# magenta/mt3

Hardware: NVIDIA B200
Metric: audio_seconds_per_second (higher is better)
Workload: dtype f32

## Files before the change

### mt3_b200/csrc/decode.cuh

```cuda
#pragma once

#include <cuda_fp16.h>

#include "common.cuh"
#include "gemm_simt.cuh"
#include "tc.cuh"

namespace mt3 {

__device__ __forceinline__ void l2_prefetch_bulk(const void* gsrc, uint32_t bytes) {
  asm volatile("cp.async.bulk.prefetch.L2.global [%0], %1;" ::"l"(reinterpret_cast<uint64_t>(gsrc)), "r"(bytes) : "memory");
}

struct DecGemmArgs {
  const float* A; int lda;
  const float* W; int ldw;
  int M, N, K;
  int norm;
  float eps;
  int epi;
  const float* R; int ldr;
  float* C; int ldc;
  int n_split; void* C1; int kv_fmt; int hm_rows_per_b; int hm_cap; int hm_H; const int* hm_pos;
  float* partial;
// ... 101 lines not shown
      *reinterpret_cast<float4*>(mine + (ty * 4 + i) * BN + tx * 4) = make_float4(acc[i][0], acc[i][1], acc[i][2], acc[i][3]);
    if ((tid & 15) == 0) {
#pragma unroll
      for (int i = 0; i < 8; ++i) mine[BM * BN + (tid >> 4) + 8 * i] = ss[i];
    }
    __threadfence();
    __syncthreads();
    if (tid == 0) {
      const int ticket = atomicAdd(&p.counters[blockIdx.x], 1);
      s_last = (ticket == splits - 1);
      if (s_last) p.counters[blockIdx.x] = 0;
    }
    __syncthreads();
    if (!s_last) return;
    __threadfence();
#pragma unroll
    for (int i = 0; i < 4; ++i)
#pragma unroll
      for (int j = 0; j < 4; ++j) acc[i][j] = 0.f;
    float sst = 0.f;
    for (int s0 = 0; s0 < splits; s0 += 4) {
      float4 v[4][4];
      float sv[4];
#pragma unroll
      for (int u = 0; u < 4; ++u) {
        const int s = s0 + u;
        const float* src = p.partial + ((long long)min(s, splits - 1) * n_tiles + blockIdx.x) * kDecTileFloats;
#pragma unroll
        for (int i = 0; i < 4; ++i) v[u][i] = __ldcg(reinterpret_cast<const float4*>(src + (ty * 4 + i) * BN + tx * 4));
        sv[u] = (tid < BM) ? __ldcg(src + BM * BN + tid) : 0.f;
      }
#pragma unroll
      for (int u = 0; u < 4; ++u) {
        if (s0 + u < splits) {
#pragma unroll
          for (int i = 0; i < 4; ++i) {
            acc[i][0] += v[u][i].x; acc[i][1] += v[u][i].y; acc[i][2] += v[u][i].z; acc[i][3] += v[u][i].w;
          }
          sst += sv[u];
        }
      }
    }
    if (tid < BM) s_ss[tid] = sst;
  } else {
    if ((tid & 15) == 0) {
#pragma unroll
      for (int i = 0; i < 8; ++i) s_ss[(tid >> 4) + 8 * i] = ss[i];
    }
  }
  __syncthreads();

#pragma unroll
  for (int i = 0; i < 4; ++i) {
    const int m = ty * 4 + i;
    if (m >= p.M) continue;
    const int n = n0 + tx * 4;
    if (n >= p.N) continue;
    const float rs = p.norm ? 1.0f / sqrtf(s_ss[m] / (float)p.K + p.eps) : 1.f;
    float4 v = make_float4(acc[i][0] * rs, acc[i][1] * rs, acc[i][2] * rs, acc[i][3] * rs);
    if (p.epi == EPI_GATED_GELU) {
      *reinterpret_cast<float2*>(p.C + (long long)m * p.ldc + (n >> 1)) = make_float2(gelu_tanh(v.x) * v.y, gelu_tanh(v.z) * v.w);
      continue;
    }
    if (p.epi == EPI_RESIDUAL) {
      const float4 q = *reinterpret_cast<const float4*>(p.R + (long long)m * p.ldr + n);
      v.x += q.x; v.y += q.y; v.z += q.z; v.w += q.w;
    }
    dec_store4(p, m, n, v);
  }
}

__device__ __forceinline__ uint32_t cluster_map(uint32_t smem_addr, unsigned rank) {
  uint32_t r;
  asm volatile("mapa.shared::cluster.u32 %0, %1, %2;" : "=r"(r) : "r"(smem_addr), "r"(rank));
  return r;
}
__device__ __forceinline__ void st_cluster_f4(uint32_t addr, float4 v) {
  asm volatile("st.shared::cluster.v4.f32 [%0], {%1, %2, %3, %4};" ::"r"(addr), "f"(v.x), "f"(v.y), "f"(v.z), "f"(v.w) : "memory");
}
__device__ __forceinline__ void st_cluster_f1(uint32_t addr, float x) {
  asm volatile("st.shared::cluster.f32 [%0], %1;" ::"r"(addr), "f"(x) : "memory");
}

constexpr int kDecLDB = kDecBN + 8;
constexpr int kDecRedFloats = 8 * 8 * kDecBN;
template <int KC, int G>
constexpr size_t dec_cluster_smem() {
  return (size_t)(kDecBM * (KC + 4) + KC * kDecLDB + kDecRedFloats + 64 + (G > 1 ? kDecBM * kDecBN : 0)) * sizeof(float);
}

template <int S>
__device__ __forceinline__ void dec_reduce_epilogue(const DecGemmArgs& p, const float* Red, const float* Rss, unsigned rank, int n0) {
  constexpr int BN = kDecBN, R = kDecBM / S, CPT = (R * BN) / 128, LPR = BN / CPT;
  static_assert(CPT == 1 || CPT == 2, "cluster size must be 8 or 16");
  const int tid = threadIdx.x;
  const int rl = tid / LPR, c0 = (tid % LPR) * CPT;
  const int m = (int)rank * R + rl, n = n0 + c0;
  float v[2] = {0.f, 0.f};
  float sst = 0.f;
#pragma unroll
  for (int s = 0; s < S; ++s) {
    if (CPT == 2) {
      const float2 q = *reinterpret_cast<const float2*>(&Red[(s * R + rl) * BN + c0]);
      v[0] += q.x; v[1] += q.y;
    } else {
      v[0] += Red[(s * R + rl) * BN + c0];
    }
    if (p.norm) sst += Rss[s * R + rl];
  }
  const bool valid = m < p.M && n < p.N;
  if (valid) {
    const float rs = p.norm ? 1.0f / sqrtf(sst / (float)p.K + p.eps) : 1.f;
    v[0] *= rs; v[1] *= rs;
    if (CPT == 2 && p.epi == EPI_GATED_GELU) {
      p.C[(long long)m * p.ldc + (n >> 1)] = gelu_tanh(v[0]) * v[1];
    } else {
      if (p.epi == EPI_RESIDUAL) {
        const float* r = p.R + (long long)m * p.ldr + n;
        v[0] += r[0];
        if (CPT == 2) v[1] += r[1];
      }
      if (n < p.n_split) {
        float* dst = p.C + (long long)m * p.ldc + n;
        if (CPT == 2) *reinterpret_cast<float2*>(dst) = make_float2(v[0], v[1]);
        else dst[0] = v[0];
      } else {
        int d;
        char* row = reinterpret_cast<char*>(p.C1) + kv_dest(m, n - p.n_split, p.hm_rows_per_b, p.hm_cap, p.hm_H, p.hm_pos ? *p.hm_pos : 0, p.kv_fmt, d);
        kv_store<CPT>(row, p.kv_fmt, d, v);
      }
    }
  }
  if (p.ssq_out) {
    float sq = valid ? fmaf(v[0], v[0], CPT == 2 ? v[1] * v[1] : 0.f) : 0.f;
#pragma unroll
    for (int o = LPR / 2; o >= 1; o >>= 1) sq += __shfl_xor_sync(0xffffffffu, sq, o);
    if ((tid % LPR) == 0 && m < p.M) p.ssq_out[(long long)m * p.ssq_ld + n0 / BN] = sq;
  }
}

template <int KC, bool TRACE, int S, int G>
__device__ __forceinline__ void dec_cluster_body(const DecGemmArgs& p, const int tile_x) {
  constexpr int BM = kDecBM, BN = kDecBN, NT = 128 * G, LDA = KC + 4, LDB = kDecLDB;
  constexpr int R = BM / S;
  constexpr int KG = KC / G;
  static_assert(KG % 4 == 0 && (KC / (2 * G)) % 4 == 0, "K chunk must split into float4 pieces per group / per ssq thread");
  extern __shared__ __align__(16) float dsm[];
  float* As = dsm;
  float* Bs = As + BM * LDA;
  float* Red = Bs + KC * LDB;
  float* Rss = Red + kDecRedFloats;
  float* Part = Rss + 64;

  unsigned rank;
  asm volatile("mov.u32 %0, %%cluster_ctarank;" : "=r"(rank));
  const int tid = threadIdx.x;
  const int grp = tid >> 7, t128 = tid & 127;
  const int n0 = tile_x * BN;
  const int kbeg = blockIdx.y * KC;
  const bool tr = TRACE && p.trace != nullptr && tid == 0;
  const bool tr0 = tr && tile_x == 0 && blockIdx.y == 0;
  long long c0 = 0;
  if (tr) {
    atomicMin(p.trace, gtime_ns());
    c0 = clock64();
    if (tile_x == 0) {
      unsigned smid;
      asm volatile("mov.u32 %0, %%smid;" : "=r"(smid));
      if (blockIdx.y < 8) p.trace[8 + blockIdx.y] = smid;
    }
  }
  asm volatile("barrier.cluster.arrive.relaxed.aligned;" ::: "memory");

  for (int idx = tid; idx < KC * 8; idx += NT) {
    const int kr = idx >> 3, nq = idx & 7;
    const bool ok = n0 + nq * 4 < p.N;
    const float* src = p.W + (long long)(kbeg + kr) * p.ldw + (ok ? n0 + nq * 4 : 0);
    asm volatile("cp.async.cg.shared.global [%0], [%1], 16, %2;" ::"r"(tc::smem_u32(&Bs[kr * LDB + nq * 4])), "l"(src),
                 "r"(ok ? 16 : 0) : "memory");
  }
  pdl_wait();
  pdl_trigger();
  for (int idx = tid; idx < KC * 16; idx += NT) {
    const int row = idx / (KC / 4), kq = idx % (KC / 4);
    const bool ok = row < p.M;
    const int col = kbeg + kq * 4;
    const float* src = (p.A2 != nullptr && col >= p.K0) ? p.A2 + (long long)(ok ? row : 0) * p.lda2 + (col - p.K0)
                                                         : p.A + (long long)(ok ? row : 0) * p.lda + col;
    asm volatile("cp.async.cg.shared.global [%0], [%1], 16, %2;" ::"r"(tc::smem_u32(&As[row * LDA + kq * 4])), "l"(src),
                 "r"(ok ? 16 : 0) : "memory");
  }
  asm volatile("cp.async.commit_group;\n\tcp.async.wait_group 0;" ::: "memory");
  __syncthreads();
  if (tr0) p.trace[2] = (unsigned long long)(clock64() - c0);

  float ss = 0.f;
  if (p.norm) {
    constexpr int PIECE = KC / (2 * G);
    const float* ar = As + (tid / (2 * G)) * LDA + (tid % (2 * G)) * PIECE;
#pragma unroll
    for (int k = 0; k < PIECE; k += 4) {
      const float4 v = *reinterpret_cast<const float4*>(ar + k);
      ss = fmaf(v.x, v.x, ss); ss = fmaf(v.y, v.y, ss); ss = fmaf(v.z, v.z, ss); ss = fmaf(v.w, v.w, ss);
    }
    ss += __shfl_xor_sync(0xffffffffu, ss, 1);
    if (G == 2) ss += __shfl_xor_sync(0xffffffffu, ss, 2);
  }

  const int tx = t128 % 8, ty = t128 / 8;
  float2 acc[4][2];
#pragma unroll
  for (int i = 0; i < 4; ++i) acc[i][0] = acc[i][1] = make_float2(0.f, 0.f);
  {
    const float* Ag = As + grp * KG;
    const float* Bg = Bs + grp * KG * LDB;
#pragma unroll 4
    for (int k = 0; k < KG; k += 4) {
      float4 a[4], b[4];
#pragma unroll
      for (int i = 0; i < 4; ++i) a[i] = *reinterpret_cast<const float4*>(&Ag[(ty + 16 * i) * LDA + k]);
#pragma unroll
      for (int kk = 0; kk < 4; ++kk) b[kk] = *reinterpret_cast<const float4*>(&Bg[(k + kk) * LDB + tx * 4]);
#pragma unroll
      for (int i = 0; i < 4; ++i) {
        const float av[4] = {a[i].x, a[i].y, a[i].z, a[i].w};
#pragma unroll
        for (int kk = 0; kk < 4; ++kk) {
          ffma2(acc[i][0], av[kk], make_float2(b[kk].x, b[kk].y));
          ffma2(acc[i][1], av[kk], make_float2(b[kk].z, b[kk].w));
        }
      }
    }
  }
  if (G == 2) {
    if (grp == 1) {
#pragma unroll
      for (int i = 0; i < 4; ++i)
        *reinterpret_cast<float4*>(&Part[(ty + 16 * i) * BN + tx * 4]) = make_float4(acc[i][0].x, acc[i][0].y, acc[i][1].x, acc[i][1].y);
    }
    __syncthreads();
    if (grp == 0) {
#pragma unroll
      for (int i = 0; i < 4; ++i) {
        const float4 q = *reinterpret_cast<const float4*>(&Part[(ty + 16 * i) * BN + tx * 4]);
        acc[i][0].x += q.x; acc[i][0].y += q.y; acc[i][1].x += q.z; acc[i][1].y += q.w;
      }
    }
  }
  if (tr0) p.trace[3] = (unsigned long long)(clock64() - c0);
  asm volatile("barrier.cluster.wait.aligned;" ::: "memory");

  const uint32_t red_base = tc::smem_u32(Red) + rank * (R * BN * 4);
  const uint32_t rss_base = tc::smem_u32(Rss) + rank * (R * 4);
  if (grp == 0) {
#pragma unroll
    for (int i = 0; i < 4; ++i) {
      const int row = ty + 16 * i;
      st_cluster_f4(cluster_map(red_base + (uint32_t)(((row % R) * BN + tx * 4) * 4), (unsigned)(row / R)),
                    make_float4(acc[i][0].x, acc[i][0].y, acc[i][1].x, acc[i][1].y));
    }
  }
  if (p.norm && (tid % (2 * G)) == 0) {
    const int row = tid / (2 * G);
    st_cluster_f1(cluster_map(rss_base + (uint32_t)((row % R) * 4), (unsigned)(row / R)), ss);
  }
  asm volatile("barrier.cluster.arrive.release.aligned;\n\tbarrier.cluster.wait.acquire.aligned;" ::: "memory");
  if (tr0) p.trace[4] = (unsigned long long)(clock64() - c0);

  if (grp == 0) dec_reduce_epilogue<S>(p, Red, Rss, rank, n0);
  if (tr) {
    if (tr0) p.trace[5] = (unsigned long long)(clock64() - c0);
    atomicMax(p.trace + 1, gtime_ns());
  }
}

template <int KC, bool TRACE, int S, int G>
__global__ void __launch_bounds__(128 * G)
sgemm_dec_cluster_kernel(const DecGemmArgs p) {
  dec_cluster_body<KC, TRACE, S, G>(p, (int)blockIdx.x);
}

template <int KC0, int KC1, bool TRACE, int G>
__global__ void __launch_bounds__(128 * G)
sgemm_dec_cluster2_kernel(const DecGemmArgs p0, const DecGemmArgs p1, const int tiles0) {
  if ((int)blockIdx.x < tiles0) dec_cluster_body<KC0, TRACE, 8, G>(p0, (int)blockIdx.x);
  else dec_cluster_body<KC1, TRACE, 8, G>(p1, (int)blockIdx.x - tiles0);
}

constexpr int kDecGroups = 1;

template <int KC0, int KC1, int G>
inline int launch_dec_gemm_cluster2_g(const DecGemmArgs& a0, const DecGemmArgs& a1, cudaStream_t s, bool pdl) {
  constexpr size_t smem = dec_cluster_smem<(KC0 > KC1 ? KC0 : KC1), G>();
  static bool attr_done = false;
  if (!attr_done) {
    MT3_CUDA_CHECK(cudaFuncSetAttribute(sgemm_dec_cluster2_kernel<KC0, KC1, false, G>, cudaFuncAttributeMaxDynamicSharedMemorySize, (int)smem));
    MT3_CUDA_CHECK(cudaFuncSetAttribute(sgemm_dec_cluster2_kernel<KC0, KC1, true, G>, cudaFuncAttributeMaxDynamicSharedMemorySize, (int)smem));
    attr_done = true;
  }
  const int tiles0 = a0.N / kDecBN, tiles1 = a1.N / kDecBN;
  if (a0.trace)
    MT3_CUDA_CHECK(launch_kernel_cluster(sgemm_dec_cluster2_kernel<KC0, KC1, true, G>, dim3(tiles0 + tiles1, 8), dim3(128 * G), smem, s,
                                         pdl, 8u, a0, a1, tiles0));
  else
    MT3_CUDA_CHECK(launch_kernel_cluster(sgemm_dec_cluster2_kernel<KC0, KC1, false, G>, dim3(tiles0 + tiles1, 8), dim3(128 * G), smem, s,
                                         pdl, 8u, a0, a1, tiles0));
  MT3_LAUNCH_CHECK();
  return MT3_OK;
}

inline int launch_dec_gemm_out_q(const DecGemmArgs& a0, const DecGemmArgs& a1, cudaStream_t s, bool pdl) {
  if (a0.M > kDecBM || a1.M > kDecBM || a0.K != 8 * 48 || a1.K != 8 * 112 || a0.N % kDecBN != 0 || a1.N % kDecBN != 0)
    return MT3_ERR_UNSUPPORTED;
  return launch_dec_gemm_cluster2_g<48, 112, kDecGroups>(a0, a1, s, pdl);
}

template <int KC, int S, int G>
inline int launch_dec_gemm_cluster_kc(const DecGemmArgs& a, cudaStream_t s, bool pdl) {
  constexpr size_t smem = dec_cluster_smem<KC, G>();
  static bool attr_done = false;
  if (!attr_done) {
    MT3_CUDA_CHECK(cudaFuncSetAttribute(sgemm_dec_cluster_kernel<KC, false, S, G>, cudaFuncAttributeMaxDynamicSharedMemorySize, (int)smem));
    MT3_CUDA_CHECK(cudaFuncSetAttribute(sgemm_dec_cluster_kernel<KC, true, S, G>, cudaFuncAttributeMaxDynamicSharedMemorySize, (int)smem));
    if (S > 8) {
      MT3_CUDA_CHECK(cudaFuncSetAttribute(sgemm_dec_cluster_kernel<KC, false, S, G>, cudaFuncAttributeNonPortableClusterSizeAllowed, 1));
      MT3_CUDA_CHECK(cudaFuncSetAttribute(sgemm_dec_cluster_kernel<KC, true, S, G>, cudaFuncAttributeNonPortableClusterSizeAllowed, 1));
    }
    attr_done = true;
  }
  if (a.trace)
    MT3_CUDA_CHECK(launch_kernel_cluster(sgemm_dec_cluster_kernel<KC, true, S, G>, dim3(cdiv(a.N, kDecBN), S), dim3(128 * G), smem, s, pdl, (unsigned)S, a));
  else
    MT3_CUDA_CHECK(launch_kernel_cluster(sgemm_dec_cluster_kernel<KC, false, S, G>, dim3(cdiv(a.N, kDecBN), S), dim3(128 * G), smem, s, pdl, (unsigned)S, a));
  MT3_LAUNCH_CHECK();
  return MT3_OK;
}

template <int G>
inline int launch_dec_gemm_cluster_g(const DecGemmArgs& a, cudaStream_t s, bool pdl) {
  if ( a.K == 1024 && a.epi != EPI_GATED_GELU && a.N <= 512) return launch_dec_gemm_cluster_kc<64, 16, G>(a, s, pdl);
  switch (a.K / 8) {
    case 48: return launch_dec_gemm_cluster_kc<48, 8, G>(a, s, pdl);
    case 64: return launch_dec_gemm_cluster_kc<64, 8, G>(a, s, pdl);
    case 128: return launch_dec_gemm_cluster_kc<128, 8, G>(a, s, pdl);
    default: return MT3_ERR_UNSUPPORTED;
  }
}

inline int launch_dec_gemm_cluster(const DecGemmArgs& a, cudaStream_t s, bool pdl) {
  if (a.M > kDecBM || a.N % 4 != 0 || a.lda % 4 != 0 || a.ldw % 4 != 0 || a.n_split % 4 != 0 || a.K % 8 != 0) return MT3_ERR_UNSUPPORTED;
  return launch_dec_gemm_cluster_g<kDecGroups>(a, s, pdl);
}

inline int launch_dec_gemm(const DecGemmArgs& a, cudaStream_t s, bool pdl = false) {
  MT3_REQUIRE(a.M <= kDecBM, MT3_ERR_UNSUPPORTED, "decode gemm: M=%d > %d rows", a.M, kDecBM);
  MT3_REQUIRE(a.K % kDecKC == 0 && a.K / kDecKC <= 16 && a.N % 4 == 0 && a.lda % 4 == 0 && a.ldw % 4 == 0 && a.n_split % 4 == 0,
              MT3_ERR_UNSUPPORTED, "decode gemm: K=%d must be a multiple of %d (at most 16 chunks); N=%d", a.K, kDecKC, a.N);
  MT3_REQUIRE(a.A2 == nullptr, MT3_ERR_UNSUPPORTED, "decode gemm: the two-source form needs the cluster kernel");
  MT3_CUDA_CHECK(launch_kernel(sgemm_dec_kernel, dim3(cdiv(a.N, kDecBN), a.K / kDecKC), dim3(128), 0, s, pdl, a));
  MT3_LAUNCH_CHECK();
  return MT3_OK;
}

constexpr int kAttRingBytes = 48 * 1024;
constexpr int kAttThreads = 160;

__device__ __forceinline__ float p24_elt(const uint4& hi, const uint2& lo, int e) {
  const uint32_t h = e < 2 ? hi.x : (e < 4 ? hi.y : (e < 6 ? hi.z : hi.w));
  const uint32_t l = e < 4 ? lo.x : lo.y;
  const uint32_t lb = 4u + (uint32_t)(e & 3);
  const uint32_t sel = (e & 1) ? (0x3200u | (lb << 4) | lb) : (0x1000u | (lb << 4) | lb);
  return __uint_as_float(__byte_perm(h, l, sel));
}

__device__ __forceinline__ uint64_t l2_evict_first_policy() {
  uint64_t pol;
  asm volatile("createpolicy.fractional.L2::evict_first.b64 %0, 1.0;" : "=l"(pol));
  return pol;
}
__device__ __forceinline__ void bulk_g2s(void* smem_dst, const void* gsrc, uint32_t bytes, uint64_t* bar, uint64_t policy) {
  asm volatile("cp.async.bulk.shared::cluster.global.mbarrier::complete_tx::bytes.L2::cache_hint [%0], [%1], %2, [%3], %4;"
               :
               : "r"(tc::smem_u32(smem_dst)), "l"(reinterpret_cast<uint64_t>(gsrc)), "r"(bytes), "r"(tc::smem_u32(bar)),
                 "l"(policy)
               : "memory");
}

inline size_t dec_attention_smem(int max_len) {
  return (size_t)kAttRingBytes + (size_t)(4 * ((max_len + 3) & ~3) + 16 * 64 + 64) * sizeof(float) + 2 * 6 * 8 + 64;
}

template <int FMT, bool TRACE>
__global__ void __launch_bounds__(kAttThreads)
dec_attention_bulk_kernel(const float* __restrict__ q, int ldq, int q_off, const void* __restrict__ kv_raw, int H, int cap,
                          const int* __restrict__ len_ptr, int len_add, int max_len, float* __restrict__ out, int ldo,
                          const float* __restrict__ q_ssq, int q_ssq_n, int q_ssq_ld, float q_dim, float q_eps,
                          unsigned long long* trace, int pf_tiles) {
  constexpr bool HALF = FMT == 1, P24 = FMT == 2;
  constexpr int KT = FMT == 0 ? 32 : 64;
  constexpr int ROWB = FMT == 0 ? 256 : (FMT == 1 ? 128 : 192);
  constexpr int kAttTileBytes = KT * ROWB;
  constexpr int kAttStages = kAttRingBytes / kAttTileBytes;
  extern __shared__ __align__(128) unsigned char sm_raw[];
  const int ml4 = (max_len + 3) & ~3;
  unsigned char* ring = sm_raw;
  float* sP = reinterpret_cast<float*>(ring + kAttStages * kAttTileBytes);
  float* sRed = sP + 4 * ml4;
  float* sQ = sRed + 16 * 64;
  uint64_t* full = reinterpret_cast<uint64_t*>(sQ + 64);
  uint64_t* empty = full + 6;
  __shared__ float s_stat[8];

  const int h = blockIdx.x, b = blockIdx.y;
  const int tid = threadIdx.x, warp = tid >> 5, lane = tid & 31;
  const int len = (len_ptr ? *len_ptr : 0) + len_add;
  const int nt = (len + KT - 1) / KT;
  const unsigned char* kbase = reinterpret_cast<const unsigned char*>(kv_raw) + (((long long)b * 2 + 0) * H + h) * (long long)cap * ROWB;
  const unsigned char* vbase = reinterpret_cast<const unsigned char*>(kv_raw) + (((long long)b * 2 + 1) * H + h) * (long long)cap * ROWB;
  const bool tr = TRACE && trace != nullptr && tid == 0;
  const bool tr0 = tr && blockIdx.x == 0 && blockIdx.y == 0;
  long long c0 = 0;
  if (tr) {
    atomicMin(trace, gtime_ns());
    c0 = clock64();
  }

  if (tid == 0) {
    for (int s = 0; s < kAttStages; ++s) {
      tc::mbar_init(&full[s], 1);
      tc::mbar_init(&empty[s], 4);
    }
    tc::fence_barrier_init();
  }
  __syncthreads();

  if (warp == 4) {
    pdl_trigger();
    if (lane == 0) {
      const uint64_t policy = l2_evict_first_policy();
      bool waited = len_ptr == nullptr;
      bool prefetched = pf_tiles <= 0;
      for (int j = 0; j < 2 * nt; ++j) {
        const int s = j % kAttStages;
        const uint32_t ph = (j / kAttStages) & 1;
        const int t = j < nt ? j : j - nt;
        if (!prefetched && (j >= kAttStages || (!waited && t == nt - 1))) {
          for (int jj = max(kAttStages, j); jj < min(kAttStages + pf_tiles, 2 * nt); ++jj) {
            const int tt = jj < nt ? jj : jj - nt;
            l2_prefetch_bulk((jj < nt ? kbase : vbase) + (long long)tt * kAttTileBytes, (uint32_t)(min(KT, len - tt * KT) * ROWB));
          }
          prefetched = true;
        }
        if (!waited && t == nt - 1) {
          pdl_wait();
          waited = true;
        }
        tc::mbar_wait(&empty[s], ph ^ 1);
        const int keys = min(KT, len - t * KT);
        const uint32_t bytes = (uint32_t)keys * ROWB;
        const unsigned char* src = (j < nt ? kbase : vbase) + (long long)t * kAttTileBytes;
        tc::mbar_arrive_expect_tx(&full[s], bytes);
        bulk_g2s(ring + s * kAttTileBytes, src, bytes, &full[s], policy);
      }
    }
    return;
  }

  pdl_wait();
  pdl_trigger();
  if (tid < 16) {
    float4 q4 = *reinterpret_cast<const float4*>(q + (long long)b * ldq + q_off + h * 64 + tid * 4);
    if (q_ssq) {
      float ssq = 0.f;
      for (int i = 0; i < q_ssq_n; ++i) ssq += __ldg(q_ssq + (long long)b * q_ssq_ld + i);
      const float rs = 1.0f / sqrtf(ssq / q_dim + q_eps);
      q4.x *= rs; q4.y *= rs; q4.z *= rs; q4.w *= rs;
    }
    reinterpret_cast<float4*>(sQ)[tid] = q4;
  }
  asm volatile("bar.sync 1, 128;" ::: "memory");
  {
    const float4* q4s = reinterpret_cast<const float4*>(sQ);
    float4 qa[4], qb[4];
#pragma unroll
    for (int jj = 0; jj < 4; ++jj) {
      if (HALF || P24) {
        const int c = (4 * (warp >> 1) + jj + (lane & 7)) & 7;
        qa[jj] = q4s[2 * c];
        qb[jj] = q4s[2 * c + 1];
      } else {
        qa[jj] = q4s[(4 * warp + jj + (lane & 7)) & 15];
      }
    }
    for (int j = 0; j < nt; ++j) {
      const int s = j % kAttStages;
      tc::mbar_wait(&full[s], (j / kAttStages) & 1);
      if (tr0 && j == 0) trace[2] = (unsigned long long)(clock64() - c0);
      const int k0 = j * KT;
      float d = 0.f;
      if (HALF) {
        const int key = (warp & 1) * 32 + lane;
        const uint4* row = reinterpret_cast<const uint4*>(ring + s * kAttTileBytes + key * ROWB);
#pragma unroll
        for (int jj = 0; jj < 4; ++jj) {
          const int c = (4 * (warp >> 1) + jj + (lane & 7)) & 7;
          const uint4 kx = row[c];
          const float2 k01 = __half22float2(*reinterpret_cast<const __half2*>(&kx.x));
// ... 48 lines not shown
    const float e = expf(sP[k] - mx);
    sP[k] = e;
    lsum += e;
  }
  lsum = warp_sum(lsum);
  if (lane == 0) s_stat[4 + warp] = lsum;
  asm volatile("bar.sync 1, 128;" ::: "memory");
  const float inv = 1.0f / (s_stat[4] + s_stat[5] + s_stat[6] + s_stat[7]);
  if (tr0) trace[4] = (unsigned long long)(clock64() - c0);

  constexpr int NG = FMT == 0 ? 8 : 16;
  if (HALF || P24) {
    const int kg = tid >> 3, d8 = tid & 7;
    float acc[8];
#pragma unroll
    for (int e = 0; e < 8; ++e) acc[e] = 0.f;
    for (int j = nt; j < 2 * nt; ++j) {
      const int s = j % kAttStages;
      tc::mbar_wait(&full[s], (j / kAttStages) & 1);
      const unsigned char* tile = ring + s * kAttTileBytes;
      const int k0 = (j - nt) * KT;
#pragma unroll
      for (int i = 0; i < 4; ++i) {
        const int kk = kg + i * 16;
        if (k0 + kk < len) {
          const float pk = sP[k0 + kk];
          const uint4 vx = *reinterpret_cast<const uint4*>(tile + kk * ROWB + d8 * 16);
          float2 v01, v23, v45, v67;
          if (P24) {
            const uint2 lo = *reinterpret_cast<const uint2*>(tile + kk * ROWB + 128 + d8 * 8);
            v01 = make_float2(p24_elt(vx, lo, 0), p24_elt(vx, lo, 1)); v23 = make_float2(p24_elt(vx, lo, 2), p24_elt(vx, lo, 3));
            v45 = make_float2(p24_elt(vx, lo, 4), p24_elt(vx, lo, 5)); v67 = make_float2(p24_elt(vx, lo, 6), p24_elt(vx, lo, 7));
          } else {
            v01 = __half22float2(*reinterpret_cast<const __half2*>(&vx.x));
            v23 = __half22float2(*reinterpret_cast<const __half2*>(&vx.y));
            v45 = __half22float2(*reinterpret_cast<const __half2*>(&vx.z));
            v67 = __half22float2(*reinterpret_cast<const __half2*>(&vx.w));
          }
          acc[0] = fmaf(pk, v01.x, acc[0]); acc[1] = fmaf(pk, v01.y, acc[1]);
          acc[2] = fmaf(pk, v23.x, acc[2]); acc[3] = fmaf(pk, v23.y, acc[3]);
          acc[4] = fmaf(pk, v45.x, acc[4]); acc[5] = fmaf(pk, v45.y, acc[5]);
          acc[6] = fmaf(pk, v67.x, acc[6]); acc[7] = fmaf(pk, v67.y, acc[7]);
        }
      }
      __syncwarp();
      if (lane == 0) tc::mbar_arrive(&empty[s]);
    }
    if (tr0) trace[5] = (unsigned long long)(clock64() - c0);
    *reinterpret_cast<float4*>(sRed + kg * 64 + d8 * 8) = make_float4(acc[0], acc[1], acc[2], acc[3]);
    *reinterpret_cast<float4*>(sRed + kg * 64 + d8 * 8 + 4) = make_float4(acc[4], acc[5], acc[6], acc[7]);
  } else {
    const int kg = tid >> 4, d4 = tid & 15;
    float4 acc = make_float4(0.f, 0.f, 0.f, 0.f);
    for (int j = nt; j < 2 * nt; ++j) {
      const int s = j % kAttStages;
      tc::mbar_wait(&full[s], (j / kAttStages) & 1);
      const float* tile = reinterpret_cast<const float*>(ring + s * kAttTileBytes);
      const int k0 = (j - nt) * KT;
#pragma unroll
      for (int i = 0; i < 4; ++i) {
        const int kk = kg + i * 8;
        if (k0 + kk < len) {
          const float pk = sP[k0 + kk];
          const float4 v = *reinterpret_cast<const float4*>(tile + kk * 64 + d4 * 4);
          acc.x = fmaf(pk, v.x, acc.x); acc.y = fmaf(pk, v.y, acc.y);
          acc.z = fmaf(pk, v.z, acc.z); acc.w = fmaf(pk, v.w, acc.w);
        }
      }
      __syncwarp();
      if (lane == 0) tc::mbar_arrive(&empty[s]);
    }
    if (tr0) trace[5] = (unsigned long long)(clock64() - c0);
    *reinterpret_cast<float4*>(sRed + kg * 64 + d4 * 4) = acc;
  }
  asm volatile("bar.sync 1, 128;" ::: "memory");
  if (tid < 64) {
    float s = 0.f;
#pragma unroll
    for (int g = 0; g < NG; ++g) s += sRed[g * 64 + tid];
    out[(long long)b * ldo + h * 64 + tid] = s * inv;
  }
  if (tr) {
    if (tr0) trace[6] = (unsigned long long)(clock64() - c0);
    atomicMax(trace + 1, gtime_ns());
  }
}

}
```

### mt3_b200/csrc/experiments/uniform_fma_probe.cu

```cuda
#include <cstdint>
__constant__ float cA[4096];
__global__ void k_const(const float4* __restrict__ W, float* __restrict__ C, int K) {
  float acc[16][4];
#pragma unroll
  for (int m = 0; m < 16; ++m)
#pragma unroll
    for (int j = 0; j < 4; ++j) acc[m][j] = 0.f;
  for (int k = 0; k < K; ++k) {
    const float4 w = W[k * 32 + threadIdx.x];
#pragma unroll
    for (int m = 0; m < 16; ++m) {
      const float a = cA[m * 256 + k];
      acc[m][0] = fmaf(a, w.x, acc[m][0]); acc[m][1] = fmaf(a, w.y, acc[m][1]);
      acc[m][2] = fmaf(a, w.z, acc[m][2]); acc[m][3] = fmaf(a, w.w, acc[m][3]);
    }
  }
#pragma unroll
  for (int m = 0; m < 16; ++m)
#pragma unroll
    for (int j = 0; j < 4; ++j) C[(m * 4 + j) * 32 + threadIdx.x] = acc[m][j];
}
__global__ void k_smem(const float4* __restrict__ W, const float* __restrict__ A, float* __restrict__ C, int K) {
  __shared__ float sA[16 * 64];
  for (int i = threadIdx.x; i < 16 * 64; i += 32) sA[i] = A[i];
  __syncwarp();
  float acc[16][4];
#pragma unroll
  for (int m = 0; m < 16; ++m)
#pragma unroll
    for (int j = 0; j < 4; ++j) acc[m][j] = 0.f;
  for (int k = 0; k < 64; ++k) {
    const float4 w = W[k * 32 + threadIdx.x];
#pragma unroll
    for (int m = 0; m < 16; ++m) {
      const float a = sA[m * 64 + k];
      acc[m][0] = fmaf(a, w.x, acc[m][0]); acc[m][1] = fmaf(a, w.y, acc[m][1]);
      acc[m][2] = fmaf(a, w.z, acc[m][2]); acc[m][3] = fmaf(a, w.w, acc[m][3]);
    }
  }
#pragma unroll
  for (int m = 0; m < 16; ++m)
#pragma unroll
    for (int j = 0; j < 4; ++j) C[(m * 4 + j) * 32 + threadIdx.x] = acc[m][j];
}
```

### mt3_b200/csrc/model.cu

```cuda
#include <string.h>
#include <math.h>
#include <string>
#include <vector>
#include <map>
#include <tuple>

#include "common.cuh"
#include "gemm_simt.cuh"
#include "gemm_tc.cuh"
#include "attention_tc.cuh"
#include "decode.cuh"
#include "layers.cuh"

namespace mt3 {

struct ParamEntry { std::string name; int64_t rows, cols, offset; };

static std::vector<ParamEntry> param_table(const mt3_model_config& c) {
  std::vector<ParamEntry> t;
  int64_t off = 0;
  auto add = [&](const std::string& n, int64_t r, int64_t co) {
    t.push_back({n, r, co, off});
    off += r * co;
  };
// ... 260 lines not shown
    const long long n4 = (long long)M * D / 4;
    split_pair_kernel<<<(unsigned)((n4 + 255) / 256), 256, 0, s>>>(encoded, m->a_enc.hi, m->a_enc.lo, n4);
    MT3_LAUNCH_CHECK();
    ope = m->a_enc.op;
  } else {
    MT3_TRY(make_operand(&ope, encoded, nullptr, M, D, D));
  }
  for (int l = 0; l < m->Ld; ++l) {
    TcGemmArgs a = tc_args(M, 2 * Q, D, nullptr, nullptr, 2 * Q);
    a.n_split = 0; a.C1 = kv_layer(m, m->ckv, l, m->T); a.kv_fmt = m->kv_fmt; a.hm_rows_per_b = m->T; a.hm_cap = m->T; a.hm_H = m->H;
    MT3_TRY(launch_tc_gemm(ope, m->dec[l].t_wkv_c.op, a, m->split3, s));
  }
  return MT3_OK;
}

static int encode_impl(Model* m, const float* x, float* encoded, cudaStream_t s) {
  if (m->tc) return encode_tc_impl(m, x, encoded, s);
  const int M = m->B * m->T, D = m->D, Q = m->Q, F = m->F;
  MT3_TRY(set_attr_once());
  {
    GemmArgs a = gemm_args(x, m->cfg.input_depth, m->w_in, D, M, D, m->cfg.input_depth, m->h, D);
    a.epi = EPI_ADD_PE; a.pe = m->pe; a.pe_T = m->T; a.pe_ld = D;
    MT3_TRY(gemm(m, a, s));
  }
  const size_t attn_smem = (size_t)(32 * kHD + 32 * (m->T + 4) + 64 * 68) * sizeof(float);
  MT3_REQUIRE(attn_smem <= 200 * 1024, MT3_ERR_UNSUPPORTED, "encode: input_length %d too long for the attention kernel", m->T);
  for (int l = 0; l < m->Le; ++l) {
    const EncLayer& w = m->enc[l];
    MT3_TRY(launch_rstd(m->h, D, M, D, m->rstd, s));
    {
      GemmArgs a = gemm_args(m->h, D, w.wqkv, 3 * Q, M, 3 * Q, D, m->qkv, 3 * Q);
      a.row_scale = m->rstd;
      MT3_TRY(gemm(m, a, s));
    }
    {
      dim3 grid(cdiv(m->T, 32), m->H, m->B);
      enc_attention_kernel<<<grid, 256, attn_smem, s>>>(m->qkv, 3 * Q, m->T, m->H, m->ao, nullptr, Q);
      MT3_LAUNCH_CHECK();
    }
    {
      GemmArgs a = gemm_args(m->ao, Q, w.wo, D, M, D, Q, m->h, D);
      a.epi = EPI_RESIDUAL; a.R = m->h; a.ldr = D;
      MT3_TRY(gemm(m, a, s));
    }
    MT3_TRY(launch_rstd(m->h, D, M, D, m->rstd, s));
    {
      GemmArgs a = gemm_args(m->h, D, w.wi, 2 * F, M, 2 * F, D, m->g, F);
      a.row_scale = m->rstd; a.epi = EPI_GATED_GELU;
      MT3_TRY(gemm(m, a, s));
    }
    {
      GemmArgs a = gemm_args(m->g, F, w.wo2, D, M, D, F, m->h, D);
      a.epi = EPI_RESIDUAL; a.R = m->h; a.ldr = D;
      MT3_TRY(gemm(m, a, s));
    }
  }
  rmsnorm_kernel<<<cdiv(M, 8), 256, 0, s>>>(m->h, nullptr, D, M, D, 1e-6f, m->enc_norm_g, encoded, D);
  MT3_LAUNCH_CHECK();
  return MT3_OK;
}

static int cross_kv_impl(Model* m, const float* encoded, cudaStream_t s) {
  const int M = m->B * m->T, D = m->D, Q = m->Q;
  if (m->tc) {
    MT3_TRY(cross_kv_tc_impl(m, encoded, s));
  } else {
    for (int l = 0; l < m->Ld; ++l) {
      GemmArgs a = gemm_args(encoded, D, m->dec[l].wkv_c, 2 * Q, M, 2 * Q, D, nullptr, 2 * Q);
      a.n_split = 0; a.C1 = kv_layer(m, m->ckv, l, m->T); a.kv_fmt = m->kv_fmt; a.hm_rows_per_b = m->T; a.hm_cap = m->T; a.hm_H = m->H;
      MT3_TRY(gemm(m, a, s));
    }
  }
  MT3_CUDA_CHECK(cudaMemsetAsync(m->state, 0, 4 * sizeof(int), s));
  MT3_CUDA_CHECK(cudaMemsetAsync(m->dcounters, 0, (size_t)m->dcounters_n * sizeof(int), s));
  MT3_CUDA_CHECK(cudaMemsetAsync(m->finished, 0, (size_t)m->B * sizeof(int), s));
  MT3_CUDA_CHECK(cudaMemsetAsync(m->tok_cur, 0, (size_t)m->B * sizeof(int), s));
  m->have_cross = true;
  m->host_pos = 0;
  return MT3_OK;
}

struct Rows { int begin, count; };

constexpr int kTraceSlots = 256, kTraceWords = 16;
static unsigned long long* trace_slot(Model* m, const char* name) {
  if (!m->tracing || (int)m->trace_names.size() >= kTraceSlots) return nullptr;
  m->trace_names.push_back(name);
  return m->trace + (size_t)(m->trace_names.size() - 1) * kTraceWords;
}

static int dec_gemm(Model* m, const float* A, int lda, const float* W, int N, int K, int norm, int epi, float* C, int ldc,
                    int n_split, char* kv, const int* pos, const Rows& rows, cudaStream_t s) {
  for (int r0 = rows.begin; r0 < rows.begin + rows.count; r0 += kDecBM) {
    DecGemmArgs a;
    memset(&a, 0, sizeof(a));
    a.A = A + (int64_t)r0 * lda; a.lda = lda; a.W = W; a.ldw = N; a.M = std::min(kDecBM, rows.begin + rows.count - r0);
    a.N = N; a.K = K;
    a.norm = norm; a.eps = 1e-6f; a.epi = epi;
    a.R = C + (int64_t)r0 * ldc; a.ldr = ldc;
    a.C = C + (int64_t)r0 * ldc; a.ldc = ldc; a.n_split = n_split;
    if (kv) {
      a.C1 = kv + (int64_t)r0 * 2 * m->H * m->L * m->kv_row; a.kv_fmt = m->kv_fmt;
      a.hm_rows_per_b = 1; a.hm_cap = m->L; a.hm_H = m->H; a.hm_pos = pos;
    }
    a.partial = m->dpartial;
    a.counters = m->dcounters;
    a.trace = trace_slot(m, K == m->F ? "gemm_mlp_out" : (N == 2 * m->F ? "gemm_mlp_in" : (kv ? "gemm_qkv_append" : (N == m->V ? "gemm_logits" : (K == m->Q ? "gemm_attn_out" : "gemm_cross_q")))));
    int rc = MT3_ERR_UNSUPPORTED;
    if (m->dec_cluster) rc = launch_dec_gemm_cluster(a, s, m->pdl_gemm);
    if (rc == MT3_ERR_UNSUPPORTED) rc = launch_dec_gemm(a, s, m->pdl_gemm);
    MT3_TRY(rc);
  }
  return MT3_OK;
}

template <int FMT>
static int launch_dec_attention_t(Model* m, const float* q, const char* kv, int cap, const int* len_ptr, int len_add,
                                  float* out, const Rows& rows, cudaStream_t s, const float* q_ssq, size_t smem, int max_len,
                                  bool prefetch) {
  static bool attr_done = false;
  if (!attr_done) {
    MT3_CUDA_CHECK(cudaFuncSetAttribute(dec_attention_bulk_kernel<FMT, false>, cudaFuncAttributeMaxDynamicSharedMemorySize, 100 * 1024));
    MT3_CUDA_CHECK(cudaFuncSetAttribute(dec_attention_bulk_kernel<FMT, true>, cudaFuncAttributeMaxDynamicSharedMemorySize, 100 * 1024));
    attr_done = true;
  }
  MT3_CUDA_CHECK(launch_kernel(m->tracing ? dec_attention_bulk_kernel<FMT, true> : dec_attention_bulk_kernel<FMT, false>,
                               dim3(m->H, rows.count), dim3(kAttThreads), smem, s, m->pdl_attn,
                               q + (int64_t)rows.begin * m->Q, m->Q, 0,
                               (const void*)(kv + (int64_t)rows.begin * 2 * m->H * cap * m->kv_row), m->H, cap,
                               len_ptr, len_add, max_len, out + (int64_t)rows.begin * m->Q, m->Q,
                               q_ssq ? q_ssq + (int64_t)rows.begin * (m->D / 32) : (const float*)nullptr, m->D / 32, m->D / 32,
                               (float)m->D, 1e-6f, trace_slot(m, len_ptr ? "attn_self" : "attn_cross"), prefetch ? m->pf_attn : 0));
  MT3_LAUNCH_CHECK();
  return MT3_OK;
}

static int launch_dec_attention(Model* m, const float* q, const char* kv, int cap, const int* len_ptr, int len_add,
                                float* out, const Rows& rows, cudaStream_t s, const float* q_ssq = nullptr, bool prefetch = false) {
  const int max_len = std::max(m->L, m->T);
  const size_t smem = dec_attention_smem(max_len);
  MT3_REQUIRE(smem <= 100 * 1024, MT3_ERR_UNSUPPORTED, "decode attention: length %d too long", max_len);
  switch (m->kv_fmt) {
    case MT3_KV_F16: return launch_dec_attention_t<1>(m, q, kv, cap, len_ptr, len_add, out, rows, s, q_ssq, smem, max_len, prefetch);
    case MT3_KV_P24: return launch_dec_attention_t<2>(m, q, kv, cap, len_ptr, len_add, out, rows, s, q_ssq, smem, max_len, prefetch);
    default: return launch_dec_attention_t<0>(m, q, kv, cap, len_ptr, len_add, out, rows, s, q_ssq, smem, max_len, prefetch);
  }
}

static int dec_gemm_out_q(Model* m, const DecLayer& w, const float* y_in, float* y_out, const Rows& rows, cudaStream_t s) {
  const int D = m->D, Q = m->Q;
  if (rows.count > kDecBM || Q != 384 || D != 512) return MT3_ERR_UNSUPPORTED;
  const int64_t r0 = rows.begin;
  DecGemmArgs a0, a1;
  memset(&a0, 0, sizeof(a0));
  a0.A = m->dao + r0 * Q; a0.lda = Q; a0.W = w.wo; a0.ldw = D; a0.M = rows.count; a0.N = D; a0.K = Q;
  a0.eps = 1e-6f; a0.epi = EPI_RESIDUAL; a0.R = y_in + r0 * D; a0.ldr = D; a0.C = y_out + r0 * D; a0.ldc = D; a0.n_split = D;
  a0.ssq_out = m->dssq + r0 * (D / 32); a0.ssq_ld = D / 32;
  a0.trace = trace_slot(m, "gemm_out+cross_q");
  memset(&a1, 0, sizeof(a1));
  a1.A = m->dao + r0 * Q; a1.lda = Q; a1.A2 = y_in + r0 * D; a1.lda2 = D; a1.K0 = Q;
  a1.W = w.wc1; a1.ldw = Q; a1.M = rows.count; a1.N = Q; a1.K = Q + D;
  a1.eps = 1e-6f; a1.epi = EPI_STORE; a1.C = m->dq + r0 * Q; a1.ldc = Q; a1.n_split = Q;
  a1.R = a1.C; a1.ldr = Q;
  a1.trace = a0.trace;
  return launch_dec_gemm_out_q(a0, a1, s, m->pdl_gemm);
}

// ... 660 lines not shown
```

Measured before the change: 288.5.

## Replace K-split thread groups with N-wide tiles in decode cluster GEMM

The decode cluster GEMM now tiles wider in N instead of splitting K across thread groups. Each 128-thread subgroup computes its own kDecBN column slice over the full K chunk and writes straight to the cluster reduction buffer, which removes the intra-CTA partial-sum pass and its barrier. The out_q fused launch now uses width 2, halving the number of tiles and sharing the A tile across two column slices, at the cost of more shared memory per CTA. General decode GEMMs still pick width 1, and extra SM-occupancy tracing counters and probe kernels are added.

```diff
diff --git a/mt3_b200/csrc/decode.cuh b/mt3_b200/csrc/decode.cuh
--- a/mt3_b200/csrc/decode.cuh
+++ b/mt3_b200/csrc/decode.cuh
@@ -207,18 +207,26 @@
   asm volatile("st.shared::cluster.f32 [%0], %1;" ::"r"(addr), "f"(x) : "memory");
 }
 
-constexpr int kDecLDB = kDecBN + 8;
 constexpr int kDecRedFloats = 8 * 8 * kDecBN;
-template <int KC, int G>
+template <int KC, int W>
 constexpr size_t dec_cluster_smem() {
-  return (size_t)(kDecBM * (KC + 4) + KC * kDecLDB + kDecRedFloats + 64 + (G > 1 ? kDecBM * kDecBN : 0)) * sizeof(float);
+  return (size_t)(kDecBM * (KC + 4) + KC * (W * kDecBN + 8) + W * kDecRedFloats + 64) * sizeof(float);
+}
+
+__device__ unsigned g_dec_sm_ctas[2][256];
+
+__device__ __forceinline__ unsigned sm_id() {
+  unsigned smid;
+  asm volatile("mov.u32 %0, %%smid;" : "=r"(smid));
+  return smid & 255u;
 }
 
 template <int S>
-__device__ __forceinline__ void dec_reduce_epilogue(const DecGemmArgs& p, const float* Red, const float* Rss, unsigned rank, int n0) {
+__device__ __forceinline__ void dec_reduce_epilogue(const DecGemmArgs& p, const float* Red, const float* Rss, unsigned rank, int n0,
+                                                    int ld = kDecBN) {
   constexpr int BN = kDecBN, R = kDecBM / S, CPT = (R * BN) / 128, LPR = BN / CPT;
   static_assert(CPT == 1 || CPT == 2, "cluster size must be 8 or 16");
-  const int tid = threadIdx.x;
+  const int tid = threadIdx.x & 127;
   const int rl = tid / LPR, c0 = (tid % LPR) * CPT;
   const int m = (int)rank * R + rl, n = n0 + c0;
   float v[2] = {0.f, 0.f};
@@ -226,10 +234,10 @@
 #pragma unroll
   for (int s = 0; s < S; ++s) {
     if (CPT == 2) {
-      const float2 q = *reinterpret_cast<const float2*>(&Red[(s * R + rl) * BN + c0]);
+      const float2 q = *reinterpret_cast<const float2*>(&Red[(s * R + rl) * ld + c0]);
       v[0] += q.x; v[1] += q.y;
     } else {
-      v[0] += Red[(s * R + rl) * BN + c0];
+      v[0] += Red[(s * R + rl) * ld + c0];
     }
     if (p.norm) sst += Rss[s * R + rl];
   }
@@ -264,41 +272,38 @@
   }
 }
 
-template <int KC, bool TRACE, int S, int G>
+template <int KC, bool TRACE, int S, int W>
 __device__ __forceinline__ void dec_cluster_body(const DecGemmArgs& p, const int tile_x) {
-  constexpr int BM = kDecBM, BN = kDecBN, NT = 128 * G, LDA = KC + 4, LDB = kDecLDB;
+  constexpr int BM = kDecBM, BN = kDecBN * W, NT = 128 * W, LDA = KC + 4, LDB = BN + 8;
   constexpr int R = BM / S;
-  constexpr int KG = KC / G;
-  static_assert(KG % 4 == 0 && (KC / (2 * G)) % 4 == 0, "K chunk must split into float4 pieces per group / per ssq thread");
+  static_assert(KC % 8 == 0, "K chunk must split into float4 pieces per ssq thread");
   extern __shared__ __align__(16) float dsm[];
   float* As = dsm;
   float* Bs = As + BM * LDA;
   float* Red = Bs + KC * LDB;
-  float* Rss = Red + kDecRedFloats;
-  float* Part = Rss + 64;
+  float* Rss = Red + W * kDecRedFloats;
 
   unsigned rank;
   asm volatile("mov.u32 %0, %%cluster_ctarank;" : "=r"(rank));
   const int tid = threadIdx.x;
-  const int grp = tid >> 7, t128 = tid & 127;
+  const int sub = tid >> 7, t128 = tid & 127;
   const int n0 = tile_x * BN;
   const int kbeg = blockIdx.y * KC;
   const bool tr = TRACE && p.trace != nullptr && tid == 0;
   const bool tr0 = tr && tile_x == 0 && blockIdx.y == 0;
   long long c0 = 0;
+  unsigned smid = 0;
   if (tr) {
     atomicMin(p.trace, gtime_ns());
     c0 = clock64();
-    if (tile_x == 0) {
-      unsigned smid;
-      asm volatile("mov.u32 %0, %%smid;" : "=r"(smid));
-      if (blockIdx.y < 8) p.trace[8 + blockIdx.y] = smid;
-    }
+    smid = sm_id();
+    atomicAdd(&g_dec_sm_ctas[0][smid], 1u);
+    if (tile_x == 0 && blockIdx.y < 8) p.trace[8 + blockIdx.y] = smid;
   }
   asm volatile("barrier.cluster.arrive.relaxed.aligned;" ::: "memory");
 
-  for (int idx = tid; idx < KC * 8; idx += NT) {
-    const int kr = idx >> 3, nq = idx & 7;
+  for (int idx = tid; idx < KC * 8 * W; idx += NT) {
+    const int kr = idx / (8 * W), nq = idx % (8 * W);
     const bool ok = n0 + nq * 4 < p.N;
     const float* src = p.W + (long long)(kbeg + kr) * p.ldw + (ok ? n0 + nq * 4 : 0);
     asm volatile("cp.async.cg.shared.global [%0], [%1], 16, %2;" ::"r"(tc::smem_u32(&Bs[kr * LDB + nq * 4])), "l"(src),
@@ -320,16 +325,15 @@
   if (tr0) p.trace[2] = (unsigned long long)(clock64() - c0);
 
   float ss = 0.f;
-  if (p.norm) {
-    constexpr int PIECE = KC / (2 * G);
-    const float* ar = As + (tid / (2 * G)) * LDA + (tid % (2 * G)) * PIECE;
+  if (p.norm && sub == 0) {
+    constexpr int PIECE = KC / 2;
+    const float* ar = As + (tid / 2) * LDA + (tid % 2) * PIECE;
 #pragma unroll
     for (int k = 0; k < PIECE; k += 4) {
       const float4 v = *reinterpret_cast<const float4*>(ar + k);
       ss = fmaf(v.x, v.x, ss); ss = fmaf(v.y, v.y, ss); ss = fmaf(v.z, v.z, ss); ss = fmaf(v.w, v.w, ss);
     }
     ss += __shfl_xor_sync(0xffffffffu, ss, 1);
-    if (G == 2) ss += __shfl_xor_sync(0xffffffffu, ss, 2);
   }
 
   const int tx = t128 % 8, ty = t128 / 8;
@@ -337,13 +341,12 @@
 #pragma unroll
   for (int i = 0; i < 4; ++i) acc[i][0] = acc[i][1] = make_float2(0.f, 0.f);
   {
-    const float* Ag = As + grp * KG;
-    const float* Bg = Bs + grp * KG * LDB;
+    const float* Bg = Bs + sub * kDecBN;
 #pragma unroll 4
-    for (int k = 0; k < KG; k += 4) {
+    for (int k = 0; k < KC; k += 4) {
       float4 a[4], b[4];
 #pragma unroll
-      for (int i = 0; i < 4; ++i) a[i] = *reinterpret_cast<const float4*>(&Ag[(ty + 16 * i) * LDA + k]);
+      for (int i = 0; i < 4; ++i) a[i] = *reinterpret_cast<const float4*>(&As[(ty + 16 * i) * LDA + k]);
 #pragma unroll
       for (int kk = 0; kk < 4; ++kk) b[kk] = *reinterpret_cast<const float4*>(&Bg[(k + kk) * LDB + tx * 4]);
 #pragma unroll
@@ -357,78 +360,70 @@
       }
     }
   }
-  if (G == 2) {
-    if (grp == 1) {
-#pragma unroll
-      for (int i = 0; i < 4; ++i)
-        *reinterpret_cast<float4*>(&Part[(ty + 16 * i) * BN + tx * 4]) = make_float4(acc[i][0].x, acc[i][0].y, acc[i][1].x, acc[i][1].y);
-    }
-    __syncthreads();
-    if (grp == 0) {
-#pragma unroll
-      for (int i = 0; i < 4; ++i) {
-        const float4 q = *reinterpret_cast<const float4*>(&Part[(ty + 16 * i) * BN + tx * 4]);
-        acc[i][0].x += q.x; acc[i][0].y += q.y; acc[i][1].x += q.z; acc[i][1].y += q.w;
-      }
-    }
-  }
-  if (tr0) p.trace[3] = (unsigned long long)(clock64() - c0);
+  if (tr) {
+    if (tr0) p.trace[3] = (unsigned long long)(clock64() - c0);
+    atomicMax(p.trace + 16, gtime_ns());
+  }
   asm volatile("barrier.cluster.wait.aligned;" ::: "memory");
 
   const uint32_t red_base = tc::smem_u32(Red) + rank * (R * BN * 4);
   const uint32_t rss_base = tc::smem_u32(Rss) + rank * (R * 4);
-  if (grp == 0) {
-#pragma unroll
-    for (int i = 0; i < 4; ++i) {
-      const int row = ty + 16 * i;
-      st_cluster_f4(cluster_map(red_base + (uint32_t)(((row % R) * BN + tx * 4) * 4), (unsigned)(row / R)),
-                    make_float4(acc[i][0].x, acc[i][0].y, acc[i][1].x, acc[i][1].y));
-    }
-  }
-  if (p.norm && (tid % (2 * G)) == 0) {
-    const int row = tid / (2 * G);
+#pragma unroll
+  for (int i = 0; i < 4; ++i) {
+    const int row = ty + 16 * i;
+    st_cluster_f4(cluster_map(red_base + (uint32_t)(((row % R) * BN + sub * kDecBN + tx * 4) * 4), (unsigned)(row / R)),
+                  make_float4(acc[i][0].x, acc[i][0].y, acc[i][1].x, acc[i][1].y));
+  }
+  if (p.norm && sub == 0 && (tid % 2) == 0) {
+    const int row = tid / 2;
     st_cluster_f1(cluster_map(rss_base + (uint32_t)((row % R) * 4), (unsigned)(row / R)), ss);
   }
   asm volatile("barrier.cluster.arrive.release.aligned;\n\tbarrier.cluster.wait.acquire.aligned;" ::: "memory");
-  if (tr0) p.trace[4] = (unsigned long long)(clock64() - c0);
-
-  if (grp == 0) dec_reduce_epilogue<S>(p, Red, Rss, rank, n0);
+  if (tr) {
+    if (tr0) p.trace[4] = (unsigned long long)(clock64() - c0);
+    const unsigned long long t = gtime_ns();
+    atomicMax(p.trace + 17, t);
+    const unsigned ng = min(*reinterpret_cast<volatile unsigned*>(&g_dec_sm_ctas[0][smid]), 255u);
+    const unsigned na = min(*reinterpret_cast<volatile unsigned*>(&g_dec_sm_ctas[1][smid]), 255u);
+    atomicMax(p.trace + 18, ((t & ((1ull << 40) - 1)) << 24) | ((unsigned long long)smid << 16) | (ng << 8) | na);
+  }
+
+  if (n0 + sub * kDecBN < p.N) dec_reduce_epilogue<S>(p, Red + sub * kDecBN, Rss, rank, n0 + sub * kDecBN, BN);
   if (tr) {
     if (tr0) p.trace[5] = (unsigned long long)(clock64() - c0);
+    atomicSub(&g_dec_sm_ctas[0][smid], 1u);
     atomicMax(p.trace + 1, gtime_ns());
   }
 }
 
-template <int KC, bool TRACE, int S, int G>
-__global__ void __launch_bounds__(128 * G)
+template <int KC, bool TRACE, int S, int W>
+__global__ void __launch_bounds__(128 * W)
 sgemm_dec_cluster_kernel(const DecGemmArgs p) {
-  dec_cluster_body<KC, TRACE, S, G>(p, (int)blockIdx.x);
-}
-
-template <int KC0, int KC1, bool TRACE, int G>
-__global__ void __launch_bounds__(128 * G)
+  dec_cluster_body<KC, TRACE, S, W>(p, (int)blockIdx.x);
+}
+
+template <int KC0, int KC1, bool TRACE, int W>
+__global__ void __launch_bounds__(128 * W)
 sgemm_dec_cluster2_kernel(const DecGemmArgs p0, const DecGemmArgs p1, const int tiles0) {
-  if ((int)blockIdx.x < tiles0) dec_cluster_body<KC0, TRACE, 8, G>(p0, (int)blockIdx.x);
-  else dec_cluster_body<KC1, TRACE, 8, G>(p1, (int)blockIdx.x - tiles0);
-}
-
-constexpr int kDecGroups = 1;
-
-template <int KC0, int KC1, int G>
-inline int launch_dec_gemm_cluster2_g(const DecGemmArgs& a0, const DecGemmArgs& a1, cudaStream_t s, bool pdl) {
-  constexpr size_t smem = dec_cluster_smem<(KC0 > KC1 ? KC0 : KC1), G>();
+  if ((int)blockIdx.x < tiles0) dec_cluster_body<KC0, TRACE, 8, W>(p0, (int)blockIdx.x);
+  else dec_cluster_body<KC1, TRACE, 8, W>(p1, (int)blockIdx.x - tiles0);
+}
+
+template <int KC0, int KC1, int W>
+inline int launch_dec_gemm_cluster2_w(const DecGemmArgs& a0, const DecGemmArgs& a1, cudaStream_t s, bool pdl) {
+  constexpr size_t smem = dec_cluster_smem<(KC0 > KC1 ? KC0 : KC1), W>();
   static bool attr_done = false;
   if (!attr_done) {
-    MT3_CUDA_CHECK(cudaFuncSetAttribute(sgemm_dec_cluster2_kernel<KC0, KC1, false, G>, cudaFuncAttributeMaxDynamicSharedMemorySize, (int)smem));
-    MT3_CUDA_CHECK(cudaFuncSetAttribute(sgemm_dec_cluster2_kernel<KC0, KC1, true, G>, cudaFuncAttributeMaxDynamicSharedMemorySize, (int)smem));
+    MT3_CUDA_CHECK(cudaFuncSetAttribute(sgemm_dec_cluster2_kernel<KC0, KC1, false, W>, cudaFuncAttributeMaxDynamicSharedMemorySize, (int)smem));
+    MT3_CUDA_CHECK(cudaFuncSetAttribute(sgemm_dec_cluster2_kernel<KC0, KC1, true, W>, cudaFuncAttributeMaxDynamicSharedMemorySize, (int)smem));
     attr_done = true;
   }
-  const int tiles0 = a0.N / kDecBN, tiles1 = a1.N / kDecBN;
+  const int tiles0 = cdiv(a0.N, W * kDecBN), tiles1 = cdiv(a1.N, W * kDecBN);
   if (a0.trace)
-    MT3_CUDA_CHECK(launch_kernel_cluster(sgemm_dec_cluster2_kernel<KC0, KC1, true, G>, dim3(tiles0 + tiles1, 8), dim3(128 * G), smem, s,
+    MT3_CUDA_CHECK(launch_kernel_cluster(sgemm_dec_cluster2_kernel<KC0, KC1, true, W>, dim3(tiles0 + tiles1, 8), dim3(128 * W), smem, s,
                                          pdl, 8u, a0, a1, tiles0));
   else
-    MT3_CUDA_CHECK(launch_kernel_cluster(sgemm_dec_cluster2_kernel<KC0, KC1, false, G>, dim3(tiles0 + tiles1, 8), dim3(128 * G), smem, s,
+    MT3_CUDA_CHECK(launch_kernel_cluster(sgemm_dec_cluster2_kernel<KC0, KC1, false, W>, dim3(tiles0 + tiles1, 8), dim3(128 * W), smem, s,
                                          pdl, 8u, a0, a1, tiles0));
   MT3_LAUNCH_CHECK();
   return MT3_OK;
@@ -437,44 +432,49 @@
 inline int launch_dec_gemm_out_q(const DecGemmArgs& a0, const DecGemmArgs& a1, cudaStream_t s, bool pdl) {
   if (a0.M > kDecBM || a1.M > kDecBM || a0.K != 8 * 48 || a1.K != 8 * 112 || a0.N % kDecBN != 0 || a1.N % kDecBN != 0)
     return MT3_ERR_UNSUPPORTED;
-  return launch_dec_gemm_cluster2_g<48, 112, kDecGroups>(a0, a1, s, pdl);
-}
-
-template <int KC, int S, int G>
+  return launch_dec_gemm_cluster2_w<48, 112, 2>(a0, a1, s, pdl);
+}
+
+template <int KC, int S, int W>
 inline int launch_dec_gemm_cluster_kc(const DecGemmArgs& a, cudaStream_t s, bool pdl) {
-  constexpr size_t smem = dec_cluster_smem<KC, G>();
+  constexpr size_t smem = dec_cluster_smem<KC, W>();
   static bool attr_done = false;
   if (!attr_done) {
-    MT3_CUDA_CHECK(cudaFuncSetAttribute(sgemm_dec_cluster_kernel<KC, false, S, G>, cudaFuncAttributeMaxDynamicSharedMemorySize, (int)smem));
-    MT3_CUDA_CHECK(cudaFuncSetAttribute(sgemm_dec_cluster_kernel<KC, true, S, G>, cudaFuncAttributeMaxDynamicSharedMemorySize, (int)smem));
+    MT3_CUDA_CHECK(cudaFuncSetAttribute(sgemm_dec_cluster_kernel<KC, false, S, W>, cudaFuncAttributeMaxDynamicSharedMemorySize, (int)smem));
+    MT3_CUDA_CHECK(cudaFuncSetAttribute(sgemm_dec_cluster_kernel<KC, true, S, W>, cudaFuncAttributeMaxDynamicSharedMemorySize, (int)smem));
     if (S > 8) {
-      MT3_CUDA_CHECK(cudaFuncSetAttribute(sgemm_dec_cluster_kernel<KC, false, S, G>, cudaFuncAttributeNonPortableClusterSizeAllowed, 1));
-      MT3_CUDA_CHECK(cudaFuncSetAttribute(sgemm_dec_cluster_kernel<KC, true, S, G>, cudaFuncAttributeNonPortableClusterSizeAllowed, 1));
+      MT3_CUDA_CHECK(cudaFuncSetAttribute(sgemm_dec_cluster_kernel<KC, false, S, W>, cudaFuncAttributeNonPortableClusterSizeAllowed, 1));
+      MT3_CUDA_CHECK(cudaFuncSetAttribute(sgemm_dec_cluster_kernel<KC, true, S, W>, cudaFuncAttributeNonPortableClusterSizeAllowed, 1));
     }
     attr_done = true;
   }
+  const dim3 grid(cdiv(a.N, W * kDecBN), S);
   if (a.trace)
-    MT3_CUDA_CHECK(launch_kernel_cluster(sgemm_dec_cluster_kernel<KC, true, S, G>, dim3(cdiv(a.N, kDecBN), S), dim3(128 * G), smem, s, pdl, (unsigned)S, a));
+    MT3_CUDA_CHECK(launch_kernel_cluster(sgemm_dec_cluster_kernel<KC, true, S, W>, grid, dim3(128 * W), smem, s, pdl, (unsigned)S, a));
   else
-    MT3_CUDA_CHECK(launch_kernel_cluster(sgemm_dec_cluster_kernel<KC, false, S, G>, dim3(cdiv(a.N, kDecBN), S), dim3(128 * G), smem, s, pdl, (unsigned)S, a));
+    MT3_CUDA_CHECK(launch_kernel_cluster(sgemm_dec_cluster_kernel<KC, false, S, W>, grid, dim3(128 * W), smem, s, pdl, (unsigned)S, a));
   MT3_LAUNCH_CHECK();
   return MT3_OK;
 }
 
-template <int G>
-inline int launch_dec_gemm_cluster_g(const DecGemmArgs& a, cudaStream_t s, bool pdl) {
-  if ( a.K == 1024 && a.epi != EPI_GATED_GELU && a.N <= 512) return launch_dec_gemm_cluster_kc<64, 16, G>(a, s, pdl);
-  switch (a.K / 8) {
-    case 48: return launch_dec_gemm_cluster_kc<48, 8, G>(a, s, pdl);
-    case 64: return launch_dec_gemm_cluster_kc<64, 8, G>(a, s, pdl);
-    case 128: return launch_dec_gemm_cluster_kc<128, 8, G>(a, s, pdl);
-    default: return MT3_ERR_UNSUPPORTED;
-  }
+inline int dec_gemm_width(const DecGemmArgs& a) {
+  return 1;
+}
+
+template <int KC, int S>
+inline int launch_dec_gemm_cluster_s(const DecGemmArgs& a, cudaStream_t s, bool pdl) {
+  return dec_gemm_width(a) == 2 ? launch_dec_gemm_cluster_kc<KC, S, 2>(a, s, pdl) : launch_dec_gemm_cluster_kc<KC, S, 1>(a, s, pdl);
 }
 
 inline int launch_dec_gemm_cluster(const DecGemmArgs& a, cudaStream_t s, bool pdl) {
   if (a.M > kDecBM || a.N % 4 != 0 || a.lda % 4 != 0 || a.ldw % 4 != 0 || a.n_split % 4 != 0 || a.K % 8 != 0) return MT3_ERR_UNSUPPORTED;
-  return launch_dec_gemm_cluster_g<kDecGroups>(a, s, pdl);
+  if (a.K == 1024 && a.epi != EPI_GATED_GELU && a.N <= 512) return launch_dec_gemm_cluster_s<64, 16>(a, s, pdl);
+  switch (a.K / 8) {
+    case 48: return launch_dec_gemm_cluster_s<48, 8>(a, s, pdl);
+    case 64: return launch_dec_gemm_cluster_s<64, 8>(a, s, pdl);
+    case 128: return launch_dec_gemm_cluster_s<128, 8>(a, s, pdl);
+    default: return MT3_ERR_UNSUPPORTED;
+  }
 }
 
 inline int launch_dec_gemm(const DecGemmArgs& a, cudaStream_t s, bool pdl = false) {
@@ -545,9 +545,12 @@
   const bool tr = TRACE && trace != nullptr && tid == 0;
   const bool tr0 = tr && blockIdx.x == 0 && blockIdx.y == 0;
   long long c0 = 0;
+  unsigned smid = 0;
   if (tr) {
     atomicMin(trace, gtime_ns());
     c0 = clock64();
+    smid = sm_id();
+    atomicAdd(&g_dec_sm_ctas[1][smid], 1u);
   }
 
   if (tid == 0) {
@@ -762,6 +765,7 @@
   }
   if (tr) {
     if (tr0) trace[6] = (unsigned long long)(clock64() - c0);
+    atomicSub(&g_dec_sm_ctas[1][smid], 1u);
     atomicMax(trace + 1, gtime_ns());
   }
 }
diff --git a/mt3_b200/csrc/experiments/uniform_fma_probe.cu b/mt3_b200/csrc/experiments/uniform_fma_probe.cu
--- a/mt3_b200/csrc/experiments/uniform_fma_probe.cu
+++ b/mt3_b200/csrc/experiments/uniform_fma_probe.cu
@@ -43,3 +43,49 @@
 #pragma unroll
     for (int j = 0; j < 4; ++j) C[(m * 4 + j) * 32 + threadIdx.x] = acc[m][j];
 }
+__global__ void k_redux(const float4* __restrict__ W, const float* __restrict__ A, float* __restrict__ C, int K) {
+  __shared__ float sA[16 * 64];
+  for (int i = threadIdx.x; i < 16 * 64; i += 32) sA[i] = A[i];
+  __syncwarp();
+  float acc[16][4];
+#pragma unroll
+  for (int m = 0; m < 16; ++m)
+#pragma unroll
+    for (int j = 0; j < 4; ++j) acc[m][j] = 0.f;
+  for (int k = 0; k < 64; ++k) {
+    const float4 w = W[k * 32 + threadIdx.x];
+#pragma unroll
+    for (int m = 0; m < 16; ++m) {
+      const float a = __uint_as_float(__reduce_or_sync(0xffffffffu, __float_as_uint(sA[m * 64 + k])));
+      acc[m][0] = fmaf(a, w.x, acc[m][0]); acc[m][1] = fmaf(a, w.y, acc[m][1]);
+      acc[m][2] = fmaf(a, w.z, acc[m][2]); acc[m][3] = fmaf(a, w.w, acc[m][3]);
+    }
+  }
+#pragma unroll
+  for (int m = 0; m < 16; ++m)
+#pragma unroll
+    for (int j = 0; j < 4; ++j) C[(m * 4 + j) * 32 + threadIdx.x] = acc[m][j];
+}
+__global__ void k_shfl(const float4* __restrict__ W, const float* __restrict__ A, float* __restrict__ C, int K) {
+  __shared__ float sA[16 * 64];
+  for (int i = threadIdx.x; i < 16 * 64; i += 32) sA[i] = A[i];
+  __syncwarp();
+  float acc[16][4];
+#pragma unroll
+  for (int m = 0; m < 16; ++m)
+#pragma unroll
+    for (int j = 0; j < 4; ++j) acc[m][j] = 0.f;
+  for (int k = 0; k < 64; ++k) {
+    const float4 w = W[k * 32 + threadIdx.x];
+#pragma unroll
+    for (int m = 0; m < 16; ++m) {
+      const float a = __shfl_sync(0xffffffffu, sA[m * 64 + k], 0);
+      acc[m][0] = fmaf(a, w.x, acc[m][0]); acc[m][1] = fmaf(a, w.y, acc[m][1]);
+      acc[m][2] = fmaf(a, w.z, acc[m][2]); acc[m][3] = fmaf(a, w.w, acc[m][3]);
+    }
+  }
+#pragma unroll
+  for (int m = 0; m < 16; ++m)
+#pragma unroll
+    for (int j = 0; j < 4; ++j) C[(m * 4 + j) * 32 + threadIdx.x] = acc[m][j];
+}
diff --git a/mt3_b200/csrc/model.cu b/mt3_b200/csrc/model.cu
--- a/mt3_b200/csrc/model.cu
+++ b/mt3_b200/csrc/model.cu
@@ -366,7 +366,7 @@
 
 struct Rows { int begin, count; };
 
-constexpr int kTraceSlots = 256, kTraceWords = 16;
+constexpr int kTraceSlots = 256, kTraceWords = 24;
 static unsigned long long* trace_slot(Model* m, const char* name) {
   if (!m->tracing || (int)m->trace_names.size() >= kTraceSlots) return nullptr;
   m->trace_names.push_back(name);
```

New measurement: 295.4, median of 6. +2.4%, better.
